# RaphaelHaddad/Real-Time-Brain-Inspired-Video-Memory

Measured on AMD Instinct MI355X. Metric: frame-embeddings/sec (+ kNN queries/sec, see knn), higher is better.
Workload: dtype f16; 1 GPU; BASELINE configs[1]: ViT-B/16-224 encoder fp16, chunks of 16 frames, cosine top-10 over a 100000-row x 768 fp16 memory shard per GPU; chunk_size=16, memory_rows_per_gpu=100000, top_k=10, parallelism=single GPU

## Files before the change

### real-time-brain-inspired-video-memory_amd/csrc/attention.hip

```cpp
#include "vm_internal.h"
#include "vm_kernels.h"

namespace {

typedef short s4v __attribute__((__vector_size__(4 * sizeof(short))));
typedef __attribute__((address_space(3))) s4v *lds_s4v_ptr;
typedef const __attribute__((address_space(3))) char *lds_cptr;

__device__ __forceinline__ bool any_above(const f32x4 a, const f32x4 b, float ref) {
    return (a[0] > ref) | (a[1] > ref) | (a[2] > ref) | (a[3] > ref) | (b[0] > ref) | (b[1] > ref) | (b[2] > ref) |
           (b[3] > ref);
}

template <class E>
__device__ __forceinline__ uint16_t ctx_value(float o, float inv) {
    float prod = o * inv;
    asm("" : "+v"(prod));
    return E::from_float(prod);
}

template <int DT, int NT, bool EXACT, bool CAUSAL = false>
__device__ __forceinline__ void attend_tile(const char *kl, const char *vl, typename vm_elem<DT>::vec8 qa,
                                            typename vm_elem<DT>::vec8 qb, int T, int lane, bool qvalid,
                                            uint16_t *dst_row, int ctx_nt = 0, int qrow = 0) {
    using E = vm_elem<DT>;
    using vec8 = typename E::vec8;
    constexpr int NS = (NT + 1) / 2;
    const int r16 = lane & 15, h = lane >> 4;
    const float scale_log2e = 0.125f * 1.44269504088896340736f;
    const int tq = r16 >> 2, tp = r16 & 3;
    f32x4 s[NT];
    float mx = -INFINITY;
#pragma unroll
    for (int kt = 0; kt < NT; ++kt) {
        const int key = kt * 16 + r16;
        const vec8 k0 = *reinterpret_cast<const vec8 *>(kl + key * 128 + ((h ^ (key & 7)) << 4));
        const vec8 k1 = *reinterpret_cast<const vec8 *>(kl + key * 128 + (((h + 4) ^ (key & 7)) << 4));
        f32x4 a = f32x4{0.f, 0.f, 0.f, 0.f};
        a = E::mfma16(k0, qa, a);
        a = E::mfma16(k1, qb, a);
        if (CAUSAL) {
#pragma unroll
            for (int j = 0; j < 4; ++j) {
                const int key = kt * 16 + 4 * h + j;
                a[j] = (key < T && key <= qrow) ? a[j] : -INFINITY;
            }
        } else if (EXACT ? (kt == NT - 1) : (kt * 16 + 16 > T)) {
#pragma unroll
            for (int j = 0; j < 4; ++j) a[j] = (kt * 16 + 4 * h + j < T) ? a[j] : -INFINITY;
        }
        mx = fmaxf(fmaxf(mx, fmaxf(a[0], a[1])), fmaxf(a[2], a[3]));
        s[kt] = a;
    }
    mx = fmaxf(mx, __shfl_xor(mx, 16, 64));
    mx = fmaxf(mx, __shfl_xor(mx, 32, 64));
    const float neg_mxc = -mx * scale_log2e;
    typedef float f32x2 __attribute__((ext_vector_type(2)));
    const f32x2 c2 = {scale_log2e, scale_log2e}, n2 = {neg_mxc, neg_mxc};
    f32x2 sum2 = {0.f, 0.f};
#pragma unroll
    for (int kt = 0; kt < NT; ++kt) {
        f32x2 a01 = __builtin_elementwise_fma(f32x2{s[kt][0], s[kt][1]}, c2, n2);
        f32x2 a23 = __builtin_elementwise_fma(f32x2{s[kt][2], s[kt][3]}, c2, n2);
        a01 = f32x2{__builtin_amdgcn_exp2f(a01.x), __builtin_amdgcn_exp2f(a01.y)};
        a23 = f32x2{__builtin_amdgcn_exp2f(a23.x), __builtin_amdgcn_exp2f(a23.y)};
        sum2 += a01;
        sum2 += a23;
        s[kt] = f32x4{a01.x, a01.y, a23.x, a23.y};
    }
    float sum = sum2.x + sum2.y;
    sum += __shfl_xor(sum, 16, 64);
    sum += __shfl_xor(sum, 32, 64);
    const float inv = 1.0f / sum;

    f32x4 o[4];
#pragma unroll
    for (int dt = 0; dt < 4; ++dt) o[dt] = f32x4{0.f, 0.f, 0.f, 0.f};
#pragma unroll
    for (int ks = 0; ks < NS; ++ks) {
        uint16_t pe[8];
#pragma unroll
        for (int j = 0; j < 4; ++j) {
            pe[j] = E::from_float(s[2 * ks][j]);
            pe[4 + j] = (2 * ks + 1 < NT) ? E::from_float(s[2 * ks + 1][j]) : (uint16_t)0;
        }
        vec8 pf;
        __builtin_memcpy(&pf, pe, 16);
        const int key_lo = ks * 32 + 4 * h + tq, key_hi = key_lo + 16;
        const char *row_lo = vl + key_lo * 128 + (tp & 1) * 8;
        const int sw = key_lo & 7;
#pragma unroll
        for (int dt = 0; dt < 4; ++dt) {
            const int coff = ((2 * dt + (tp >> 1)) ^ sw) << 4;
            const s4v lo = __builtin_amdgcn_ds_read_tr16_b64_v4i16((lds_s4v_ptr)(row_lo + coff));
            const s4v hi = __builtin_amdgcn_ds_read_tr16_b64_v4i16(
                (lds_s4v_ptr)(row_lo + (2 * ks + 1 < NT ? 16 * 128 : 0) + coff));
            typedef short s8v __attribute__((__vector_size__(8 * sizeof(short))));
            const s8v av = __builtin_shufflevector(lo, hi, 0, 1, 2, 3, 4, 5, 6, 7);
            o[dt] = E::mfma16(__builtin_bit_cast(vec8, av), pf, o[dt]);
        }
        (void)key_hi;
    }
    if (qvalid) {
        uint16_t *dst = dst_row + 4 * h;
#pragma unroll
        for (int dt = 0; dt < 4; ++dt) {
            uint16_t oe[4];
#pragma unroll
            for (int j = 0; j < 4; ++j) oe[j] = ctx_value<E>(o[dt][j], inv);
            uint2 pk;
            __builtin_memcpy(&pk, oe, 8);
            typedef unsigned ctx_u32x2 __attribute__((ext_vector_type(2)));
            if (ctx_nt) __builtin_nontemporal_store(ctx_u32x2{pk.x, pk.y}, reinterpret_cast<ctx_u32x2 *>(dst + dt * 16));
            else *reinterpret_cast<uint2 *>(dst + dt * 16) = pk;
        }
    }
}

template <int DT, int NT, bool EXACT>
__device__ __forceinline__ float attend_rowmax(const char *kl, typename vm_elem<DT>::vec8 qa,
                                               typename vm_elem<DT>::vec8 qb, int T, int lane) {
    using E = vm_elem<DT>;
    using vec8 = typename E::vec8;
    const int r16 = lane & 15, h = lane >> 4;
    const char *p0 = kl + r16 * 128 + ((h ^ (r16 & 7)) << 4);
    const char *p1 = kl + r16 * 128 + (((h + 4) ^ (r16 & 7)) << 4);
    auto tile = [&](int kt, bool masked) {
        const vec8 k0 = *reinterpret_cast<const vec8 *>(p0 + kt * 2048);
        const vec8 k1 = *reinterpret_cast<const vec8 *>(p1 + kt * 2048);
        f32x4 a = f32x4{0.f, 0.f, 0.f, 0.f};
        a = E::mfma16(k0, qa, a);
        a = E::mfma16(k1, qb, a);
        if (masked) {
#pragma unroll
            for (int j = 0; j < 4; ++j) a[j] = (kt * 16 + 4 * h + j < T) ? a[j] : -INFINITY;
        }
        return fmaxf(fmaxf(a[0], a[1]), fmaxf(a[2], a[3]));
    };
    float mx0 = -INFINITY, mx1 = -INFINITY;
    constexpr int FULL = EXACT ? NT - 1 : 0;
    int kt = 0;
#pragma unroll 1
    for (; kt + 1 < FULL; kt += 2) {
        mx0 = fmaxf(mx0, tile(kt, false));
        mx1 = fmaxf(mx1, tile(kt + 1, false));
    }
#pragma unroll 1
    for (; kt < NT; ++kt) mx0 = fmaxf(mx0, tile(kt, kt >= FULL));
    float mx = fmaxf(mx0, mx1);
    mx = fmaxf(mx, __shfl_xor(mx, 16, 64));
    mx = fmaxf(mx, __shfl_xor(mx, 32, 64));
    return mx;
}

template <int DT, int NT, bool EXACT, bool ONLINE = false>
__device__ __forceinline__ void attend_tile_pass2(const char *kl, const char *vl, typename vm_elem<DT>::vec8 qa,
                                                  typename vm_elem<DT>::vec8 qb, float mx, int T, int lane,
                                                  bool qvalid, uint16_t *dst_row) {
    using E = vm_elem<DT>;
    using vec8 = typename E::vec8;
    typedef float f32x2 __attribute__((ext_vector_type(2)));
    typedef short s8v __attribute__((__vector_size__(8 * sizeof(short))));
    constexpr int NS = (NT + 1) / 2;
    const int r16 = lane & 15, h = lane >> 4;
    const int tq = r16 >> 2, tp = r16 & 3;
    const float scale_log2e = 0.125f * 1.44269504088896340736f;
    constexpr float ONLINE_SLACK = 6.0f;
    float run_m = ONLINE ? -1e30f : mx;
    float run_hi = -1e30f;
    float neg_mxc = -run_m * scale_log2e;
    const f32x2 c2 = {scale_log2e, scale_log2e};
    f32x2 n2 = {neg_mxc, neg_mxc};
    const char *p0 = kl + r16 * 128 + ((h ^ (r16 & 7)) << 4);
    const char *p1 = kl + r16 * 128 + (((h + 4) ^ (r16 & 7)) << 4);
    const int vsw = (4 * h + tq) & 7;
    const char *vrow = vl + (4 * h + tq) * 128 + (tp & 1) * 8;
    int voff[4];
#pragma unroll
    for (int dt = 0; dt < 4; ++dt) voff[dt] = ((2 * dt + (tp >> 1)) ^ vsw) << 4;
    f32x2 sum2 = {0.f, 0.f};
    f32x4 o[4];
#pragma unroll
    for (int dt = 0; dt < 4; ++dt) o[dt] = f32x4{0.f, 0.f, 0.f, 0.f};

    lds_cptr kp0 = (lds_cptr)p0, kp1 = (lds_cptr)p1;
    lds_cptr vp[4];
#pragma unroll
    for (int dt = 0; dt < 4; ++dt) vp[dt] = (lds_cptr)(vrow + voff[dt]);
    auto step = [&](int ks, bool masked0, bool has1, bool masked1) {
        const int hi_off = has1 ? 16 * 128 : 0;
        typedef const __attribute__((address_space(3))) vec8 *lds_vec8_ptr;
        const vec8 ka0 = *(lds_vec8_ptr)(kp0);
        const vec8 ka1 = *(lds_vec8_ptr)(kp1);
        const vec8 kb0 = *(lds_vec8_ptr)(kp0 + (has1 ? 2048 : 0));
        const vec8 kb1 = *(lds_vec8_ptr)(kp1 + (has1 ? 2048 : 0));
        s4v vlo[4], vhi[4];
#pragma unroll
        for (int dt = 0; dt < 4; ++dt) {
            vlo[dt] = __builtin_amdgcn_ds_read_tr16_b64_v4i16((lds_s4v_ptr)(vp[dt]));
            vhi[dt] = __builtin_amdgcn_ds_read_tr16_b64_v4i16((lds_s4v_ptr)(vp[dt] + hi_off));
        }
        kp0 += 4096;
        kp1 += 4096;
#pragma unroll
        for (int dt = 0; dt < 4; ++dt) vp[dt] += 4096;
        asm volatile("" : "+v"(kp0), "+v"(kp1), "+v"(vp[0]), "+v"(vp[1]), "+v"(vp[2]), "+v"(vp[3]));
        f32x4 a[2];
        a[0] = E::mfma16(ka0, qa, f32x4{0.f, 0.f, 0.f, 0.f});
        a[0] = E::mfma16(ka1, qb, a[0]);
        a[1] = E::mfma16(kb0, qa, f32x4{0.f, 0.f, 0.f, 0.f});
        a[1] = E::mfma16(kb1, qb, a[1]);
        if (masked0) {
#pragma unroll
            for (int j = 0; j < 4; ++j) a[0][j] = ((2 * ks) * 16 + 4 * h + j < T) ? a[0][j] : -INFINITY;
        }
        if (!has1) {
            a[1] = f32x4{-INFINITY, -INFINITY, -INFINITY, -INFINITY};
        } else if (masked1) {
#pragma unroll
            for (int j = 0; j < 4; ++j) a[1][j] = ((2 * ks + 1) * 16 + 4 * h + j < T) ? a[1][j] : -INFINITY;
        }
        if (ONLINE) {
            if (__ballot(any_above(a[0], a[1], run_hi)) != 0ull) {
                const float lm_own = fmaxf(fmaxf(fmaxf(a[0][0], a[0][1]), fmaxf(a[0][2], a[0][3])),
                                           fmaxf(fmaxf(a[1][0], a[1][1]), fmaxf(a[1][2], a[1][3])));
                float lm = fmaxf(lm_own, __shfl_xor(lm_own, 16, 64));
                lm = fmaxf(lm, __shfl_xor(lm, 32, 64));
                const float m_new = fmaxf(run_m, lm);
                const float f = __builtin_amdgcn_exp2f((run_m - m_new) * scale_log2e);
                sum2 *= f32x2{f, f};
#pragma unroll
                for (int dt = 0; dt < 4; ++dt) o[dt] *= f32x4{f, f, f, f};
                run_m = m_new;
                run_hi = run_m + ONLINE_SLACK / scale_log2e;
                neg_mxc = -run_m * scale_log2e;
                n2 = f32x2{neg_mxc, neg_mxc};
            }
        }
        uint16_t pe[8];
#pragma unroll
        for (int u = 0; u < 2; ++u) {
            f32x2 p01 = __builtin_elementwise_fma(f32x2{a[u][0], a[u][1]}, c2, n2);
            f32x2 p23 = __builtin_elementwise_fma(f32x2{a[u][2], a[u][3]}, c2, n2);
            p01 = f32x2{__builtin_amdgcn_exp2f(p01.x), __builtin_amdgcn_exp2f(p01.y)};
            p23 = f32x2{__builtin_amdgcn_exp2f(p23.x), __builtin_amdgcn_exp2f(p23.y)};
            sum2 += p01 + p23;
            pe[4 * u + 0] = E::from_float(p01.x);
            pe[4 * u + 1] = E::from_float(p01.y);
            pe[4 * u + 2] = E::from_float(p23.x);
            pe[4 * u + 3] = E::from_float(p23.y);
        }
        vec8 pf;
        __builtin_memcpy(&pf, pe, 16);
#pragma unroll
        for (int dt = 0; dt < 4; ++dt) {
            const s8v av = __builtin_shufflevector(vlo[dt], vhi[dt], 0, 1, 2, 3, 4, 5, 6, 7);
            o[dt] = E::mfma16(__builtin_bit_cast(vec8, av), pf, o[dt]);
        }
    };
    constexpr int FULL_STEPS = EXACT ? (NT - 1) / 2 : 0;
    int ks = 0;
#pragma unroll 1
    for (; ks < FULL_STEPS; ++ks) step(ks, false, true, false);
#pragma unroll 1
    for (; ks < NS; ++ks) step(ks, true, 2 * ks + 1 < NT, true);

    float sum = sum2.x + sum2.y;
    sum += __shfl_xor(sum, 16, 64);
    sum += __shfl_xor(sum, 32, 64);
    const float inv = 1.0f / sum;
    if (qvalid) {
        uint16_t *dst = dst_row + 4 * h;
#pragma unroll
        for (int dt = 0; dt < 4; ++dt) {
            uint16_t oe[4];
#pragma unroll
            for (int j = 0; j < 4; ++j) oe[j] = ctx_value<E>(o[dt][j], inv);
            uint2 pk;
            __builtin_memcpy(&pk, oe, 8);
            *reinterpret_cast<uint2 *>(dst + dt * 16) = pk;
        }
    }
}

__device__ __forceinline__ void wait_vmcnt_dyn(int n) {
#define VM_W(N) case N: asm volatile("s_waitcnt vmcnt(" #N ")" ::: "memory"); break;
    switch (n) {
        VM_W(1) VM_W(2) VM_W(3) VM_W(4) VM_W(5) VM_W(6) VM_W(7) VM_W(8) VM_W(9) VM_W(10) VM_W(11) VM_W(12) VM_W(13)
        VM_W(14) VM_W(15) VM_W(16) VM_W(17) VM_W(18) VM_W(19) VM_W(20) VM_W(21) VM_W(22) VM_W(23) VM_W(24) VM_W(25)
        VM_W(26) VM_W(27) VM_W(28) VM_W(29) VM_W(30) VM_W(31) VM_W(32) VM_W(33) VM_W(34) VM_W(35) VM_W(36) VM_W(37)
        VM_W(38) VM_W(39) VM_W(40) VM_W(41) VM_W(42) VM_W(43) VM_W(44) VM_W(45) VM_W(46) VM_W(47) VM_W(48)
        default: asm volatile("s_waitcnt vmcnt(0)" ::: "memory"); break;
    }
#undef VM_W
}

template <int DT, int NT, bool EXACT, int ABL = 0>
__device__ __forceinline__ void attend_pair_online(const char *kl, const char *vl,
                                                   const typename vm_elem<DT>::vec8 (&qa)[2],
                                                   const typename vm_elem<DT>::vec8 (&qb)[2], int T, int lane,
                                                   const bool (&qvalid)[2], uint16_t *const (&dst_row)[2]) {
    using E = vm_elem<DT>;
    using vec8 = typename E::vec8;
    typedef float f32x2 __attribute__((ext_vector_type(2)));
    constexpr int NS = (NT + 1) / 2;
    constexpr float ONLINE_SLACK = 6.0f;
    const int r16 = lane & 15, h = lane >> 4;
    const int tq = r16 >> 2, tp = r16 & 3;
    const float scale_log2e = 0.125f * 1.44269504088896340736f;
    const f32x2 c2 = {scale_log2e, scale_log2e};
    const char *p0 = kl + r16 * 128 + ((h ^ (r16 & 7)) << 4);
    const char *p1 = kl + r16 * 128 + (((h + 4) ^ (r16 & 7)) << 4);
    const int vsw = (4 * h + tq) & 7;
    const char *vrow = vl + (4 * h + tq) * 128 + (tp & 1) * 8;
    int voff[4];
#pragma unroll
    for (int dt = 0; dt < 4; ++dt) voff[dt] = ((2 * dt + (tp >> 1)) ^ vsw) << 4;
    float run_m[2] = {-1e30f, -1e30f}, run_hi[2] = {-1e30f, -1e30f};
    f32x2 n2[2] = {{1e30f * scale_log2e, 1e30f * scale_log2e}, {1e30f * scale_log2e, 1e30f * scale_log2e}};
    f32x2 sum2[2] = {{0.f, 0.f}, {0.f, 0.f}};
    f32x4 o[2][4];
#pragma unroll
    for (int t = 0; t < 2; ++t)
#pragma unroll
        for (int dt = 0; dt < 4; ++dt) o[t][dt] = f32x4{0.f, 0.f, 0.f, 0.f};

    lds_cptr kp0 = (lds_cptr)p0, kp1 = (lds_cptr)p1;
    lds_cptr vp[4];
#pragma unroll
    for (int dt = 0; dt < 4; ++dt) vp[dt] = (lds_cptr)(vrow + voff[dt]);
    auto step = [&](int ks, bool masked0, bool has1, bool masked1) {
        const int hi_off = has1 ? 16 * 128 : 0;
        typedef const __attribute__((address_space(3))) vec8 *lds_vec8_ptr;
        vec8 ka0, ka1, kb0, kb1;
        if (ABL & 32) {
            ka0 = ka1 = qa[0];
            kb0 = kb1 = qb[0];
        } else {
            ka0 = *(lds_vec8_ptr)(kp0);
            ka1 = *(lds_vec8_ptr)(kp1);
            kb0 = *(lds_vec8_ptr)(kp0 + (has1 ? 2048 : 0));
            kb1 = *(lds_vec8_ptr)(kp1 + (has1 ? 2048 : 0));
        }
        s4v vlo[4], vhi[4];
#pragma unroll
        for (int dt = 0; dt < 4; ++dt) {
            if (ABL & 16) {
                vlo[dt] = vhi[dt] = __builtin_bit_cast(s4v, (unsigned long long)(0x3c003c003c003c00ull + dt));
            } else {
                vlo[dt] = __builtin_amdgcn_ds_read_tr16_b64_v4i16((lds_s4v_ptr)(vp[dt]));
                vhi[dt] = __builtin_amdgcn_ds_read_tr16_b64_v4i16((lds_s4v_ptr)(vp[dt] + hi_off));
            }
        }
        kp0 += 4096;
        kp1 += 4096;
#pragma unroll
        for (int dt = 0; dt < 4; ++dt) vp[dt] += 4096;
        asm volatile("" : "+v"(kp0), "+v"(kp1), "+v"(vp[0]), "+v"(vp[1]), "+v"(vp[2]), "+v"(vp[3]));
        f32x4 a[2][2];
        bool out_of_slack = false;
#pragma unroll
        for (int t = 0; t < 2; ++t) {
            if (ABL & 8) {
                const f32x4 ua = __builtin_bit_cast(f32x4, ka0), ub = __builtin_bit_cast(f32x4, kb0);
                a[t][0] = f32x4{1.f, 2.f, 3.f, 4.f} + f32x4{ua[0] * 0.f, 0.f, 0.f, 0.f};
                a[t][1] = f32x4{4.f, 3.f, 2.f, 1.f} + f32x4{ub[0] * 0.f, 0.f, 0.f, 0.f};
                asm volatile("" : "+v"(a[t][0]), "+v"(a[t][1]) : "v"(ka1), "v"(kb1));
            } else {
                a[t][0] = E::mfma16(ka0, qa[t], f32x4{0.f, 0.f, 0.f, 0.f});
                a[t][0] = E::mfma16(ka1, qb[t], a[t][0]);
                a[t][1] = E::mfma16(kb0, qa[t], f32x4{0.f, 0.f, 0.f, 0.f});
                a[t][1] = E::mfma16(kb1, qb[t], a[t][1]);
            }
        }
#pragma unroll
        for (int t = 0; t < 2; ++t) {
            if (masked0) {
#pragma unroll
                for (int j = 0; j < 4; ++j) a[t][0][j] = ((2 * ks) * 16 + 4 * h + j < T) ? a[t][0][j] : -INFINITY;
            }
            if (!has1) {
                a[t][1] = f32x4{-INFINITY, -INFINITY, -INFINITY, -INFINITY};
            } else if (masked1) {
#pragma unroll
                for (int j = 0; j < 4; ++j) a[t][1][j] = ((2 * ks + 1) * 16 + 4 * h + j < T) ? a[t][1][j] : -INFINITY;
            }
            out_of_slack |= any_above(a[t][0], a[t][1], run_hi[t]);
        }
        if (__ballot(out_of_slack) != 0ull) {
#pragma unroll
            for (int t = 0; t < 2; ++t) {
                const float lm_own = fmaxf(fmaxf(fmaxf(a[t][0][0], a[t][0][1]), fmaxf(a[t][0][2], a[t][0][3])),
                                           fmaxf(fmaxf(a[t][1][0], a[t][1][1]), fmaxf(a[t][1][2], a[t][1][3])));
                float lm = fmaxf(lm_own, __shfl_xor(lm_own, 16, 64));
                lm = fmaxf(lm, __shfl_xor(lm, 32, 64));
                const float m_new = lm > run_hi[t] ? lm : run_m[t];
                const float f = __builtin_amdgcn_exp2f((run_m[t] - m_new) * scale_log2e);
                sum2[t] *= f32x2{f, f};
#pragma unroll
                for (int dt = 0; dt < 4; ++dt) o[t][dt] *= f32x4{f, f, f, f};
                run_m[t] = m_new;
                run_hi[t] = m_new + ONLINE_SLACK / scale_log2e;
                const float neg = -m_new * scale_log2e;
                n2[t] = f32x2{neg, neg};
            }
        }
        auto softmax_pack = [&](int t) -> vec8 {
            uint16_t pe[8];
#pragma unroll
            for (int u = 0; u < 2; ++u) {
                f32x2 p01 = __builtin_elementwise_fma(f32x2{a[t][u][0], a[t][u][1]}, c2, n2[t]);
                f32x2 p23 = __builtin_elementwise_fma(f32x2{a[t][u][2], a[t][u][3]}, c2, n2[t]);
                if (!(ABL & 1)) {
                    p01 = f32x2{__builtin_amdgcn_exp2f(p01.x), __builtin_amdgcn_exp2f(p01.y)};
                    p23 = f32x2{__builtin_amdgcn_exp2f(p23.x), __builtin_amdgcn_exp2f(p23.y)};
                }
                sum2[t] += p01 + p23;
                pe[4 * u + 0] = E::from_float(p01.x);
                pe[4 * u + 1] = E::from_float(p01.y);
                pe[4 * u + 2] = E::from_float(p23.x);
                pe[4 * u + 3] = E::from_float(p23.y);
            }
            vec8 pf;
            __builtin_memcpy(&pf, pe, 16);
            return pf;
        };
        vec8 av[4];
#pragma unroll
        for (int dt = 0; dt < 4; ++dt)
            av[dt] = __builtin_bit_cast(vec8, __builtin_shufflevector(vlo[dt], vhi[dt], 0, 1, 2, 3, 4, 5, 6, 7));
        const vec8 pf0 = softmax_pack(0);
        if (ABL & 2) {
            asm volatile("" ::"v"(pf0), "v"(av[0]), "v"(av[1]), "v"(av[2]), "v"(av[3]));
        } else {
#pragma unroll
            for (int dt = 0; dt < 4; ++dt) o[0][dt] = E::mfma16(av[dt], pf0, o[0][dt]);
        }
        const vec8 pf1 = softmax_pack(1);
        if (ABL & 2) {
            asm volatile("" ::"v"(pf1));
        } else {
#pragma unroll
            for (int dt = 0; dt < 4; ++dt) o[1][dt] = E::mfma16(av[dt], pf1, o[1][dt]);
        }
#pragma unroll
        for (int k = 0; k < 4; ++k) {
            __builtin_amdgcn_sched_group_barrier(0x008, 1, 0);
            __builtin_amdgcn_sched_group_barrier(0x400, 2, 0);
        }
    };
    constexpr int FULL_STEPS = EXACT ? (NT - 1) / 2 : 0;
    int ks = 0;
#pragma unroll 1
    for (; ks < FULL_STEPS; ++ks) step(ks, false, true, false);
#pragma unroll 1
    for (; ks < NS; ++ks) step(ks, true, 2 * ks + 1 < NT, true);

#pragma unroll
    for (int t = 0; t < 2; ++t) {
        float sum = sum2[t].x + sum2[t].y;
        sum += __shfl_xor(sum, 16, 64);
        sum += __shfl_xor(sum, 32, 64);
        const float inv = 1.0f / sum;
        if (qvalid[t]) {
            uint16_t *dst = dst_row[t] + 4 * h;
#pragma unroll
            for (int dt = 0; dt < 4; ++dt) {
                uint16_t oe[4];
#pragma unroll
                for (int j = 0; j < 4; ++j) oe[j] = ctx_value<E>(o[t][dt][j], inv);
                uint2 pk;
                __builtin_memcpy(&pk, oe, 8);
                *reinterpret_cast<uint2 *>(dst + dt * 16) = pk;
            }
        }
    }
}

template <int DT, int NT, bool EXACT, int NW, int ABL = 0>
__global__ void __launch_bounds__(NW * 64, 1)
    attention_pair_kernel(const uint16_t *__restrict__ qkv, uint16_t *__restrict__ ctx_out, int T, int heads,
                          int qt_lim) {
    using E = vm_elem<DT>;
    using vec8 = typename E::vec8;
    constexpr int ROWS = NT * 16;
    extern __shared__ __attribute__((aligned(16))) char smem[];
    char *kl = smem, *vl = smem + (size_t)ROWS * 128;
    const int tid = threadIdx.x, lane = tid & 63, wave = tid >> 6;
    const int r16 = lane & 15, h = lane >> 4;
    const int b = blockIdx.x / heads, head = blockIdx.x - b * heads;
    const int H = heads * 64;
    const size_t M = (size_t)(gridDim.x / heads) * T;
    auto block = [&](int part) { return qkv + ((size_t)(part * heads + head) * M + (size_t)b * T) * 64; };
    auto load_q = [&](int qt, vec8 &q0, vec8 &q1) {
        int qtok = qt * 16 + r16;
        if (qtok > T - 1) qtok = T - 1;
        const uint16_t *qp = block(0) + (size_t)qtok * 64;
        q0 = __builtin_bit_cast(vec8, *reinterpret_cast<const uint4 *>(qp + 8 * h));
        q1 = __builtin_bit_cast(vec8, *reinterpret_cast<const uint4 *>(qp + 32 + 8 * h));
    };
    const int srow = lane >> 3, scp = lane & 7;
    auto stage = [&](int part, char *dst) {
        const char *src = reinterpret_cast<const char *>(block(part));
#pragma unroll 4
        for (int grp = wave; grp < ROWS / 8; grp += NW) {
            int key = grp * 8 + srow;
            key = key > T - 1 ? T - 1 : key;
            __builtin_amdgcn_global_load_lds((gbl_ptr_t)(src + (size_t)key * 128 + ((scp ^ srow) << 4)),
                                             (lds_ptr_t)(dst + grp * 1024), 16, 0, 2);
        }
    };
    const int npairs = (qt_lim + 1) / 2;
    vec8 qa[2], qb[2];
    if (wave < npairs) {
        load_q(2 * wave, qa[0], qb[0]);
        load_q(2 * wave + 1, qa[1], qb[1]);
    }
    if (!(ABL & 4)) {
        stage(1, kl);
        stage(2, vl);
    }
    asm volatile("s_waitcnt vmcnt(0)" ::: "memory");
    __syncthreads();
    for (int pr = wave; pr < npairs; pr += NW) {
        bool qvalid[2];
        uint16_t *dst[2];
#pragma unroll
        for (int t = 0; t < 2; ++t) {
            const int qt = 2 * pr + t;
            const int qtok = qt * 16 + r16;
            qvalid[t] = qt < qt_lim && qtok < T;
            dst[t] = ctx_out + ((size_t)b * T + (qvalid[t] ? qtok : 0)) * H + head * 64;
        }
        const vec8 ca[2] = {qa[0], qa[1]}, cb[2] = {qb[0], qb[1]};
        if (pr + NW < npairs) {
            load_q(2 * (pr + NW), qa[0], qb[0]);
            load_q(2 * (pr + NW) + 1, qa[1], qb[1]);
        }
        attend_pair_online<DT, NT, EXACT, ABL>(kl, vl, ca, cb, T, lane, qvalid, dst);
    }
}

template <int DT, int NT, bool EXACT, int NW, int PF_MAX>
__global__ void __launch_bounds__(NW * 64, 1)
    attention_pair_persist_kernel(const uint16_t *__restrict__ qkv, uint16_t *__restrict__ ctx_out, int T, int heads,
                                  int qt_lim, int items) {
    using E = vm_elem<DT>;
    using vec8 = typename E::vec8;
    constexpr int ROWS = NT * 16;
    constexpr int CHUNKS = 2 * ROWS * 8;
    extern __shared__ __attribute__((aligned(16))) char smem[];
    char *kl = smem, *vl = smem + (size_t)ROWS * 128;
    const int tid = threadIdx.x, lane = tid & 63;
    const int wave = __builtin_amdgcn_readfirstlane(tid >> 6);
    const int r16 = lane & 15, h = lane >> 4;
    const int H = heads * 64;
    const size_t M = (size_t)(items / heads) * T;
    if ((int)blockIdx.x >= items) return;
    auto block = [&](int item, int part) {
        const int b = item / heads, head = item - b * heads;
        return qkv + ((size_t)(part * heads + head) * M + (size_t)b * T) * 64;
    };
    auto load_q = [&](int item, int qt, vec8 &q0, vec8 &q1) {
        int qtok = qt * 16 + r16;
        if (qtok > T - 1) qtok = T - 1;
        const uint16_t *qp = block(item, 0) + (size_t)qtok * 64;
        q0 = __builtin_bit_cast(vec8, *reinterpret_cast<const uint4 *>(qp + 8 * h));
        q1 = __builtin_bit_cast(vec8, *reinterpret_cast<const uint4 *>(qp + 32 + 8 * h));
    };
    const int npairs = (qt_lim + 1) / 2;
    const int maxc = (npairs + NW - 1) / NW;
    int w0 = npairs - (maxc - 1) * NW;
    if (w0 >= NW) w0 = 0;
    const int P = NW - w0, pw = wave - w0;

    int item = blockIdx.x;
    vec8 qa[2], qb[2];
    if (wave < npairs) {
        load_q(item, 2 * wave, qa[0], qb[0]);
        load_q(item, 2 * wave + 1, qa[1], qb[1]);
    }
    {
        const int srow = lane >> 3, scp = lane & 7;
#pragma unroll
        for (int part = 1; part <= 2; ++part) {
            const char *src = reinterpret_cast<const char *>(block(item, part));
            char *dst = part == 1 ? kl : vl;
#pragma unroll 4
            for (int grp = wave; grp < ROWS / 8; grp += NW) {
                int key = grp * 8 + srow;
                key = key > T - 1 ? T - 1 : key;
                __builtin_amdgcn_global_load_lds((gbl_ptr_t)(src + (size_t)key * 128 + ((scp ^ srow) << 4)),
                                                 (lds_ptr_t)(dst + grp * 1024), 16, 0, 2);
            }
        }
        asm volatile("s_waitcnt vmcnt(0)" ::: "memory");
        __syncthreads();
    }
    while (true) {
        const int next = item + (int)gridDim.x;
        const bool has_next = next < items;
        const int b = item / heads, head = item - b * heads;
        for (int pr = wave; pr < npairs; pr += NW) {
            bool qvalid[2];
            uint16_t *dst[2];
#pragma unroll
            for (int t = 0; t < 2; ++t) {
                const int qt = 2 * pr + t;
                const int qtok = qt * 16 + r16;
                qvalid[t] = qt < qt_lim && qtok < T;
                dst[t] = ctx_out + ((size_t)b * T + (qvalid[t] ? qtok : 0)) * H + head * 64;
            }
            const vec8 ca[2] = {qa[0], qa[1]}, cb[2] = {qb[0], qb[1]};
            if (pr + NW < npairs) {
                load_q(item, 2 * (pr + NW), qa[0], qb[0]);
                load_q(item, 2 * (pr + NW) + 1, qa[1], qb[1]);
            } else if (has_next && pw < 0) {
                load_q(next, 2 * wave, qa[0], qb[0]);
                load_q(next, 2 * wave + 1, qa[1], qb[1]);
            }
            attend_pair_online<DT, NT, EXACT, 0>(kl, vl, ca, cb, T, lane, qvalid, dst);
        }
        if (!has_next) break;
        if (pw >= 0) {
            typedef unsigned pf_u32x4 __attribute__((ext_vector_type(4)));
            pf_u32x4 buf[PF_MAX];
            const char *kbase = reinterpret_cast<const char *>(block(next, 1));
            const char *vbase = reinterpret_cast<const char *>(block(next, 2));
            int lrow = lane >> 3;
            asm volatile("" : "+v"(lrow));
            const unsigned lane_term = (unsigned)(((lane & 7) ^ lrow) << 4);
#pragma unroll
            for (int j = 0; j < PF_MAX; ++j) {
                int g = __builtin_amdgcn_readfirstlane(j * P + pw);
                g = g < CHUNKS / 64 ? g : CHUNKS / 64 - 1;
                const bool is_v = g >= ROWS / 8;
                int key = (is_v ? g - ROWS / 8 : g) * 8 + lrow;
                key = key > T - 1 ? T - 1 : key;
                const char *src = (is_v ? vbase : kbase) + ((unsigned)key * 128u + lane_term);
                buf[j] = __builtin_nontemporal_load(reinterpret_cast<const pf_u32x4 *>(src));
            }
            asm volatile("s_waitcnt lgkmcnt(0)\n\ts_barrier" ::: "memory");
#pragma unroll
            for (int j = 0; j < PF_MAX; ++j) {
                int g = __builtin_amdgcn_readfirstlane(j * P + pw);
                g = g < CHUNKS / 64 ? g : CHUNKS / 64 - 1;
                *reinterpret_cast<pf_u32x4 *>(smem + (size_t)g * 1024 + lane * 16) = buf[j];
            }
            if (wave < npairs) {
                load_q(next, 2 * wave, qa[0], qb[0]);
                load_q(next, 2 * wave + 1, qa[1], qb[1]);
            }
            asm volatile("s_waitcnt lgkmcnt(0)\n\ts_barrier" ::: "memory");
        } else {
            asm volatile("s_waitcnt lgkmcnt(0)\n\ts_barrier" ::: "memory");
            asm volatile("s_waitcnt lgkmcnt(0)\n\ts_barrier" ::: "memory");
        }
        item = next;
    }
}

template <int DT, int NT, bool EXACT, int NW, bool ONLINE>
__global__ void __launch_bounds__(NW * 64, 1)
    attention_long_kernel(const uint16_t *__restrict__ qkv, uint16_t *__restrict__ ctx_out, int T, int heads,
                          int qt_lim) {
    using E = vm_elem<DT>;
    using vec8 = typename E::vec8;
    constexpr int ROWS = NT * 16;
    extern __shared__ __attribute__((aligned(16))) char smem[];
    char *kl = smem, *vl = smem + (size_t)ROWS * 128;

    const int tid = threadIdx.x, lane = tid & 63, wave = tid >> 6;
    const int r16 = lane & 15, h = lane >> 4;
    const int b = blockIdx.x / heads, head = blockIdx.x - b * heads;
    const int H = heads * 64;
    const size_t M = (size_t)(gridDim.x / heads) * T;
    auto block = [&](int part) { return qkv + ((size_t)(part * heads + head) * M + (size_t)b * T) * 64; };
    auto load_q = [&](int qt, vec8 &q0, vec8 &q1) {
        int qtok = qt * 16 + r16;
        if (qtok > T - 1) qtok = T - 1;
        const uint16_t *qp = block(0) + (size_t)qtok * 64;
        q0 = __builtin_bit_cast(vec8, *reinterpret_cast<const uint4 *>(qp + 8 * h));
        q1 = __builtin_bit_cast(vec8, *reinterpret_cast<const uint4 *>(qp + 32 + 8 * h));
    };
    const int srow = lane >> 3, scp = lane & 7;
    auto stage = [&](int part, char *dst) {
        const char *src = reinterpret_cast<const char *>(block(part));
#pragma unroll 4
        for (int grp = wave; grp < ROWS / 8; grp += NW) {
            int key = grp * 8 + srow;
            key = key > T - 1 ? T - 1 : key;
            __builtin_amdgcn_global_load_lds((gbl_ptr_t)(src + (size_t)key * 128 + ((scp ^ srow) << 4)),
                                             (lds_ptr_t)(dst + grp * 1024), 16, 0, 2);
        }
    };
    vec8 q0, q1;
    load_q(wave, q0, q1);
    stage(1, kl);
    asm volatile("s_waitcnt vmcnt(0)" ::: "memory");
    __syncthreads();
    stage(2, vl);
    float mx = 0.f;
    if (!ONLINE && wave < qt_lim) mx = attend_rowmax<DT, NT, EXACT>(kl, q0, q1, T, lane);
    asm volatile("s_waitcnt vmcnt(0)" ::: "memory");
    __syncthreads();
    for (int qt = wave; qt < qt_lim; qt += NW) {
        const int qtok = qt * 16 + r16;
        const bool qvalid = qtok < T;
        const vec8 qa = q0, qb = q1;
        if (qt + NW < qt_lim) load_q(qt + NW, q0, q1);
        if (!ONLINE && qt != wave) mx = attend_rowmax<DT, NT, EXACT>(kl, qa, qb, T, lane);
        attend_tile_pass2<DT, NT, EXACT, ONLINE>(kl, vl, qa, qb, mx, T, lane, qvalid,
                                         ctx_out + ((size_t)b * T + (qvalid ? qtok : 0)) * H + head * 64);
    }
}

template <int DT, int NT, bool EXACT>
int launch_long(vm_ctx *ctx, const uint16_t *qkv, uint16_t *out, int B, int T, int heads, hipStream_t st, int qt_lim) {
    const size_t lds = (size_t)NT * 16 * 128 * 2;
    static const int online_env = (int)VM_DEV_ENV("ATTN_ONLINE", 1);
    static const int pair_env = (int)VM_DEV_ENV("ATTN_PAIR", 12);
    vm_prof_scope prof(ctx, VM_PROF_ATTENTION, st);
    if (online_env && pair_env > 0) {
        const int ql = qt_lim < NT ? qt_lim : NT;
#define VM_PAIR_GO(NWV)                                                                                              \
    {                                                                                                                \
        auto kern = attention_pair_kernel<DT, NT, EXACT, NWV>;                                                       \
        static unsigned long long attr_set = 0;                                               \
        if (!((attr_set >> (ctx->device & 63)) & 1ull)) {                                                                                             \
            VM_HIP(ctx, hipFuncSetAttribute((const void *)kern, hipFuncAttributeMaxDynamicSharedMemorySize, (int)lds)); \
            attr_set |= 1ull << (ctx->device & 63);                                                                                         \
        }                                                                                                            \
        kern<<<B * heads, NWV * 64, lds, st>>>(qkv, out, T, heads, ql);                                              \
    }
#ifdef VM_DEV_SWITCHES
        static const int abl_env = (int)VM_DEV_ENV("ATTN_ABL", 0);
#define VM_PAIR_ABL(A)                                                                                               \
    if (abl_env == (A)) {                                                                                            \
        auto kern = attention_pair_kernel<DT, NT, EXACT, 12, (A)>;                                                   \
        (void)hipFuncSetAttribute((const void *)kern, hipFuncAttributeMaxDynamicSharedMemorySize, (int)lds);        \
        kern<<<B * heads, 12 * 64, lds, st>>>(qkv, out, T, heads, ql);                                               \
        VM_LAUNCH_CHECK(ctx);                                                                                        \
        return VM_OK;                                                                                                \
    }
        if constexpr (NT == 37 && DT == VM_BF16) {
            VM_PAIR_ABL(1) VM_PAIR_ABL(2) VM_PAIR_ABL(4) VM_PAIR_ABL(8) VM_PAIR_ABL(16) VM_PAIR_ABL(32) VM_PAIR_ABL(3)
            VM_PAIR_ABL(10) VM_PAIR_ABL(48) VM_PAIR_ABL(63)
        }
#undef VM_PAIR_ABL
#endif
        static const int persist_env = (int)VM_DEV_ENV("ATTN_PERSIST", 1);
        const int npairs = (ql + 1) / 2, maxc = (npairs + 11) / 12;
        int w0 = npairs - (maxc - 1) * 12;
        if (w0 >= 12) w0 = 0;
        constexpr int GROUPS = 2 * NT * 16 / 8;
        constexpr int PF_FEW = (GROUPS + 4) / 5;
        constexpr int PF_MANY = (GROUPS + 10) / 11;
        const int pf = (GROUPS + (12 - w0) - 1) / (12 - w0);
        const int items = B * heads;
#define VM_PERSIST_GO(PF)                                                                                            \
    {                                                                                                                \
        auto kern = attention_pair_persist_kernel<DT, NT, EXACT, 12, PF>;                                            \
        static unsigned long long attr_set = 0;                                               \
        if (!((attr_set >> (ctx->device & 63)) & 1ull)) {                                                            \
            VM_HIP(ctx, hipFuncSetAttribute((const void *)kern, hipFuncAttributeMaxDynamicSharedMemorySize, (int)lds)); \
            attr_set |= 1ull << (ctx->device & 63);                                                                  \
        }                                                                                                            \
        kern<<<items < ctx->num_cus ? items : ctx->num_cus, 12 * 64, lds, st>>>(qkv, out, T, heads, ql, items);      \
    }
        if (persist_env && pair_env == 12 && pf <= PF_MANY) VM_PERSIST_GO(PF_MANY)
        else if (persist_env && pair_env == 12 && pf <= PF_FEW) VM_PERSIST_GO(PF_FEW)
#undef VM_PERSIST_GO
        else if (pair_env == 8) VM_PAIR_GO(8)
        else if (pair_env == 10) VM_PAIR_GO(10)
        else VM_PAIR_GO(12)
#undef VM_PAIR_GO
    } else if (online_env) {
        auto kern = attention_long_kernel<DT, NT, EXACT, 16, true>;
        static unsigned long long attr_set = 0;
        if (!((attr_set >> (ctx->device & 63)) & 1ull)) {
            VM_HIP(ctx, hipFuncSetAttribute((const void *)kern, hipFuncAttributeMaxDynamicSharedMemorySize, (int)lds));
            attr_set |= 1ull << (ctx->device & 63);
        }
        kern<<<B * heads, 1024, lds, st>>>(qkv, out, T, heads, qt_lim < NT ? qt_lim : NT);
    } else {
        auto kern = attention_long_kernel<DT, NT, EXACT, 16, false>;
        static unsigned long long attr_set = 0;
        if (!((attr_set >> (ctx->device & 63)) & 1ull)) {
            VM_HIP(ctx, hipFuncSetAttribute((const void *)kern, hipFuncAttributeMaxDynamicSharedMemorySize, (int)lds));
            attr_set |= 1ull << (ctx->device & 63);
        }
        kern<<<B * heads, 1024, lds, st>>>(qkv, out, T, heads, qt_lim < NT ? qt_lim : NT);
    }
    VM_LAUNCH_CHECK(ctx);
    return VM_OK;
}

template <int DT, int NT, bool EXACT, int OCC, bool CAUSAL = false>
__global__ void __launch_bounds__(256, OCC)
    attention_kernel(const uint16_t *__restrict__ qkv, uint16_t *__restrict__ ctx_out, int T, int heads, int qt_lim) {
    using E = vm_elem<DT>;
    using vec8 = typename E::vec8;
    constexpr int KROWS = NT * 16;
    constexpr int VROWS = KROWS;
    extern __shared__ __attribute__((aligned(16))) char smem[];
    char *kl = smem;
    char *vl = smem + (size_t)KROWS * 128;

    const int tid = threadIdx.x, lane = tid & 63, wave = tid >> 6;
    const int r16 = lane & 15, h = lane >> 4;
    const int b = blockIdx.x / heads, head = blockIdx.x - b * heads;
    const int H = heads * 64;
    const size_t M = (size_t)(gridDim.x / heads) * T;
    auto block = [&](int part) { return qkv + ((size_t)(part * heads + head) * M + (size_t)b * T) * 64; };

    auto load_q = [&](int qt, vec8 &q0, vec8 &q1) {
        int qtok = qt * 16 + r16;
        if (qtok > T - 1) qtok = T - 1;
        const uint16_t *qp = block(0) + (size_t)qtok * 64;
        q0 = __builtin_bit_cast(vec8, *reinterpret_cast<const uint4 *>(qp + 8 * h));
        q1 = __builtin_bit_cast(vec8, *reinterpret_cast<const uint4 *>(qp + 32 + 8 * h));
    };
    vec8 q0, q1;
    load_q(wave, q0, q1);
    {
        constexpr int GROUPS = (KROWS + VROWS) / 8;
        const int srow = lane >> 3, scp = lane & 7;
#pragma unroll
        for (int gi = 0; gi < (GROUPS + 3) / 4; ++gi) {
            const int grp = gi * 4 + wave;
            if (grp < GROUPS) {
                const int r = grp * 8 + srow;
                const bool is_v = r >= KROWS;
                int key = is_v ? r - KROWS : r;
                if (key > T - 1) key = T - 1;
                const uint16_t *src = block(is_v ? 2 : 1) + (size_t)key * 64 + ((scp ^ (r & 7)) << 3);
                __builtin_amdgcn_global_load_lds((gbl_ptr_t)src, (lds_ptr_t)(smem + grp * 1024), 16, 0, 0);
            }
        }
        asm volatile("s_waitcnt vmcnt(0)" ::: "memory");
    }
    __syncthreads();

    for (int qt = wave; qt < qt_lim; qt += 4) {
        const int qtok = qt * 16 + r16;
        const bool qvalid = qtok < T;
        const vec8 qa = q0, qb = q1;
        if (qt + 4 < qt_lim) load_q(qt + 4, q0, q1);

        attend_tile<DT, NT, EXACT, CAUSAL>(kl, vl, qa, qb, T, lane, qvalid,
                                           ctx_out + ((size_t)b * T + (qvalid ? qtok : 0)) * H + head * 64, 0, qtok);
    }
}

template <int DT, int NT, bool EXACT, int CW>
__global__ void __launch_bounds__((CW + 1) * 64, 1)
    attention_stream_kernel(const uint16_t *__restrict__ qkv, uint16_t *__restrict__ ctx_out, int T, int heads,
                            int items, int qt_lim, int ctx_nt) {
    using E = vm_elem<DT>;
    using vec8 = typename E::vec8;
    constexpr int ROWS = NT * 16;
    constexpr int IMG = 3 * ROWS * 128;
    constexpr int QT = (NT + CW - 1) / CW;
    extern __shared__ __attribute__((aligned(16))) char smem[];

    const int tid = threadIdx.x, lane = tid & 63, wave = tid >> 6;
    const int H = heads * 64;
    if (blockIdx.x >= items) return;

    if (wave == CW) {
        const int srow = lane >> 3, scp = lane & 7;
        const unsigned lane_off = (unsigned)((scp ^ srow) << 4);
        const size_t M = (size_t)(items / heads) * T;
        const int tmax = T - 1;
        int buf = 0;
        for (int item = blockIdx.x; item < items; item += gridDim.x, buf ^= 1) {
            const int b = item / heads, head = item - b * heads;
#pragma unroll
            for (int part = 0; part < 3; ++part) {
                const char *pbase = reinterpret_cast<const char *>(
                    qkv + ((size_t)((part == 2 ? 0 : part + 1) * heads + head) * M + (size_t)b * T) * 64);
#pragma unroll
                for (int g = 0; g < ROWS / 8; ++g) {
                    if (part == 2 && g >= 2 * qt_lim) break;
                    int key = g * 8 + srow;
                    if (!EXACT || g * 8 + 7 >= 16 * (NT - 1)) key = key > tmax ? tmax : key;
                    const unsigned off = (unsigned)key * 128 + lane_off;
                    __builtin_amdgcn_global_load_lds((gbl_ptr_t)(pbase + off),
                                                     (lds_ptr_t)(smem + buf * IMG + (part * (ROWS / 8) + g) * 1024), 16,
                                                     0, 2);
                    if ((g & 3) == 3) asm volatile("s_waitcnt vmcnt(24)" ::: "memory");
                }
            }
            asm volatile("s_waitcnt vmcnt(0)" ::: "memory");
            asm volatile("s_barrier" ::: "memory");
        }
        return;
    }

    const int r16 = lane & 15, h = lane >> 4;
    int buf = 0;
    for (int item = blockIdx.x; item < items; item += gridDim.x, buf ^= 1) {
        asm volatile("s_barrier" ::: "memory");
        const char *kl = smem + buf * IMG, *vl = kl + ROWS * 128, *ql = vl + ROWS * 128;
        const int b = item / heads, head = item - b * heads;
#pragma unroll
        for (int u = 0; u < QT; ++u) {
            const int qt = wave + CW * u;
            if (qt < qt_lim) {
                const int qtok = qt * 16 + r16;
                const bool qvalid = qtok < T;
                const vec8 qa = *reinterpret_cast<const vec8 *>(ql + qtok * 128 + ((h ^ (qtok & 7)) << 4));
                const vec8 qb = *reinterpret_cast<const vec8 *>(ql + qtok * 128 + (((h + 4) ^ (qtok & 7)) << 4));
                attend_tile<DT, NT, EXACT>(kl, vl, qa, qb, T, lane, qvalid,
                                           ctx_out + ((size_t)b * T + (qvalid ? qtok : 0)) * H + head * 64, ctx_nt);
            }
        }
    }
}

template <int DT, int NT, bool EXACT, int CW>
int launch_stream_cw(vm_ctx *ctx, const uint16_t *qkv, uint16_t *out, int B, int T, int heads, hipStream_t st, int qt_lim) {
    const size_t lds = (size_t)NT * 16 * 128 * 6;
    auto kern = attention_stream_kernel<DT, NT, EXACT, CW>;
    static unsigned long long attr_set = 0;
    if (!((attr_set >> (ctx->device & 63)) & 1ull)) {
        VM_HIP(ctx, hipFuncSetAttribute((const void *)kern, hipFuncAttributeMaxDynamicSharedMemorySize, (int)lds));
        attr_set |= 1ull << (ctx->device & 63);
    }
    const int items = B * heads;
    const int grid = items < ctx->num_cus ? items : ctx->num_cus;
    vm_prof_scope prof(ctx, VM_PROF_ATTENTION, st);
    static const int ctx_nt_env = (int)VM_DEV_ENV("ATTN_CTX_NT", 1);
    kern<<<grid, (CW + 1) * 64, lds, st>>>(qkv, out, T, heads, items, qt_lim < NT ? qt_lim : NT, ctx_nt_env);
    VM_LAUNCH_CHECK(ctx);
    return VM_OK;
}

template <int DT, int NT, bool EXACT>
int launch_stream(vm_ctx *ctx, const uint16_t *qkv, uint16_t *out, int B, int T, int heads, hipStream_t st, int qt_lim) {
    static const int cw_env = (int)VM_DEV_ENV("ATTN_CW", 13);
    if (cw_env == 8) return launch_stream_cw<DT, NT, EXACT, 8>(ctx, qkv, out, B, T, heads, st, qt_lim);
    return launch_stream_cw<DT, NT, EXACT, 13>(ctx, qkv, out, B, T, heads, st, qt_lim);
}


template <int DT, int NT, bool EXACT, int OCC = (NT <= 13 ? 2 : 1), bool CAUSAL = false>
int launch(vm_ctx *ctx, const uint16_t *qkv, uint16_t *out, int B, int T, int heads, hipStream_t st, int qt_lim) {
    const size_t lds = (size_t)NT * 16 * 128 * 2;
    auto kern = attention_kernel<DT, NT, EXACT, OCC, CAUSAL>;
    static unsigned long long attr_set = 0;
    if (!((attr_set >> (ctx->device & 63)) & 1ull)) {
        VM_HIP(ctx, hipFuncSetAttribute((const void *)kern, hipFuncAttributeMaxDynamicSharedMemorySize, (int)lds));
        attr_set |= 1ull << (ctx->device & 63);
    }
    vm_prof_scope prof(ctx, VM_PROF_ATTENTION, st);
    kern<<<B * heads, 256, lds, st>>>(qkv, out, T, heads, qt_lim < NT ? qt_lim : NT);
    VM_LAUNCH_CHECK(ctx);
    return VM_OK;
}

template <int DT>
int dispatch(vm_ctx *ctx, const uint16_t *qkv, uint16_t *out, int B, int T, int heads, hipStream_t st, int q_rows,
             int causal) {
    const int nt = (T + 15) / 16;
    if (causal) {
        if (nt > 5) return vm_fail(ctx, VM_ERR_UNSUPPORTED, "causal attention: %d tokens > 80", T);
        return launch<DT, 5, false, 2, true>(ctx, qkv, out, B, T, heads, st, 5);
    }
    const int ql = q_rows > 0 ? (q_rows + 15) / 16 : nt;
    if (nt == 13) {
        return launch_stream<DT, 13, true>(ctx, qkv, out, B, T, heads, st, ql);
    }
    if (nt == 37) return launch_long<DT, 37, true>(ctx, qkv, out, B, T, heads, st, ql);
    if (nt <= 2) return launch<DT, 2, false>(ctx, qkv, out, B, T, heads, st, ql);
    if (nt <= 5) return launch<DT, 5, false>(ctx, qkv, out, B, T, heads, st, ql);
    if (nt <= 13) return launch<DT, 13, false>(ctx, qkv, out, B, T, heads, st, ql);
    if (nt <= 37) return launch_long<DT, 37, false>(ctx, qkv, out, B, T, heads, st, ql);
    return vm_fail(ctx, VM_ERR_UNSUPPORTED, "attention: %d tokens > 592", T);
}

}

int vm_attention(vm_ctx *ctx, int dtype, const uint16_t *qkv, uint16_t *ctx_out, int B, int T, int heads,
                 hipStream_t st, int q_rows, int causal) {
    return dtype == VM_F16 ? dispatch<VM_F16>(ctx, qkv, ctx_out, B, T, heads, st, q_rows, causal)
                           : dispatch<VM_BF16>(ctx, qkv, ctx_out, B, T, heads, st, q_rows, causal);
}
```

Measured before the change: 26600 frame-embeddings/s.

## Stage attention context in LDS and drain it from the producer wave

The streaming attention kernel's producer wave now fills only K and V into LDS. Each compute wave loads its own Q tile straight from global memory, prefetching the next item's Q. Compute waves write their context output into a swizzled LDS staging buffer instead of global memory. The producer wave then drains that buffer to global with coalesced 16-byte stores while it fills the next item, and the vmcnt throttling window during fill becomes a template parameter that defaults to off. The aim is to cut scattered 8-byte global stores from the compute waves and overlap output writeback with the next load, at the cost of one wave doing both load and store work plus extra barriers.

```diff
diff --git a/real-time-brain-inspired-video-memory_amd/csrc/attention.hip b/real-time-brain-inspired-video-memory_amd/csrc/attention.hip
--- a/real-time-brain-inspired-video-memory_amd/csrc/attention.hip
+++ b/real-time-brain-inspired-video-memory_amd/csrc/attention.hip
@@ -19,7 +19,7 @@
     return E::from_float(prod);
 }
 
-template <int DT, int NT, bool EXACT, bool CAUSAL = false>
+template <int DT, int NT, bool EXACT, bool CAUSAL = false, bool LDS_CTX = false>
 __device__ __forceinline__ void attend_tile(const char *kl, const char *vl, typename vm_elem<DT>::vec8 qa,
                                             typename vm_elem<DT>::vec8 qb, int T, int lane, bool qvalid,
                                             uint16_t *dst_row, int ctx_nt = 0, int qrow = 0) {
@@ -111,6 +111,12 @@
             uint2 pk;
             __builtin_memcpy(&pk, oe, 8);
             typedef unsigned ctx_u32x2 __attribute__((ext_vector_type(2)));
+            if constexpr (LDS_CTX) {
+                typedef __attribute__((address_space(3))) ctx_u32x2 *lds_ctx_ptr;
+                char *row = reinterpret_cast<char *>(dst_row);
+                *(lds_ctx_ptr)(row + (((2 * dt + (h >> 1)) ^ (qrow & 7)) << 4) + (h & 1) * 8) = ctx_u32x2{pk.x, pk.y};
+                continue;
+            }
             if (ctx_nt) __builtin_nontemporal_store(ctx_u32x2{pk.x, pk.y}, reinterpret_cast<ctx_u32x2 *>(dst + dt * 16));
             else *reinterpret_cast<uint2 *>(dst + dt * 16) = pk;
         }
@@ -853,76 +859,121 @@
     }
 }
 
-template <int DT, int NT, bool EXACT, int CW>
+template <int DT, int NT, bool EXACT, int CW, int WIN>
 __global__ void __launch_bounds__((CW + 1) * 64, 1)
     attention_stream_kernel(const uint16_t *__restrict__ qkv, uint16_t *__restrict__ ctx_out, int T, int heads,
                             int items, int qt_lim, int ctx_nt) {
     using E = vm_elem<DT>;
     using vec8 = typename E::vec8;
     constexpr int ROWS = NT * 16;
-    constexpr int IMG = 3 * ROWS * 128;
-    constexpr int QT = (NT + CW - 1) / CW;
+    constexpr int IMG = 2 * ROWS * 128;
+    constexpr int CIMG = ROWS * 128;
+    static_assert(NT <= CW, "one query tile per compute wave");
+    static_assert(WIN >= 0 && WIN < 64, "the window must fit the vmcnt field");
     extern __shared__ __attribute__((aligned(16))) char smem[];
+    typedef unsigned st_u32x4 __attribute__((ext_vector_type(4)));
 
     const int tid = threadIdx.x, lane = tid & 63, wave = tid >> 6;
     const int H = heads * 64;
     if (blockIdx.x >= items) return;
+    const size_t M = (size_t)(items / heads) * T;
 
     if (wave == CW) {
         const int srow = lane >> 3, scp = lane & 7;
         const unsigned lane_off = (unsigned)((scp ^ srow) << 4);
-        const size_t M = (size_t)(items / heads) * T;
         const int tmax = T - 1;
-        int buf = 0;
-        for (int item = blockIdx.x; item < items; item += gridDim.x, buf ^= 1) {
+        const int row_lim = qt_lim * 16 < T ? qt_lim * 16 : T;
+        auto fill = [&](int item, int buf) {
             const int b = item / heads, head = item - b * heads;
 #pragma unroll
-            for (int part = 0; part < 3; ++part) {
+            for (int part = 0; part < 2; ++part) {
                 const char *pbase = reinterpret_cast<const char *>(
-                    qkv + ((size_t)((part == 2 ? 0 : part + 1) * heads + head) * M + (size_t)b * T) * 64);
+                    qkv + ((size_t)((part + 1) * heads + head) * M + (size_t)b * T) * 64);
 #pragma unroll
                 for (int g = 0; g < ROWS / 8; ++g) {
-                    if (part == 2 && g >= 2 * qt_lim) break;
                     int key = g * 8 + srow;
                     if (!EXACT || g * 8 + 7 >= 16 * (NT - 1)) key = key > tmax ? tmax : key;
                     const unsigned off = (unsigned)key * 128 + lane_off;
                     __builtin_amdgcn_global_load_lds((gbl_ptr_t)(pbase + off),
                                                      (lds_ptr_t)(smem + buf * IMG + (part * (ROWS / 8) + g) * 1024), 16,
                                                      0, 2);
-                    if ((g & 3) == 3) asm volatile("s_waitcnt vmcnt(24)" ::: "memory");
+                    if (WIN > 0 && (g & 3) == 3) asm volatile("s_waitcnt vmcnt(%0)" ::"n"(WIN) : "memory");
                 }
             }
-            asm volatile("s_waitcnt vmcnt(0)" ::: "memory");
-            asm volatile("s_barrier" ::: "memory");
-        }
+        };
+        auto drain = [&](int item, int buf) {
+            const int b = item / heads, head = item - b * heads;
+            int grp_bytes = H * 16;
+            asm volatile("" : "+s"(grp_bytes));
+            char *obase = reinterpret_cast<char *>(ctx_out + ((size_t)b * T * H + (size_t)head * 64));
+            const unsigned lane_dst = (unsigned)srow * ((unsigned)grp_bytes >> 3) + lane_off;
+            const char *img = smem + 2 * IMG + buf * CIMG + lane * 16;
+            constexpr int GB = NT;
+            for (int g0 = 0; g0 < 2 * GB && g0 * 8 < row_lim; g0 += GB) {
+                st_u32x4 v[GB];
+#pragma unroll
+                for (int j = 0; j < GB; ++j)
+                    v[j] = *reinterpret_cast<const __attribute__((address_space(3))) st_u32x4 *>(
+                        (lds_cptr)(img + (g0 + j) * 1024));
+#pragma unroll
+                for (int j = 0; j < GB; ++j) {
+                    if ((g0 + j) * 8 + srow < row_lim) {
+                        st_u32x4 *dst = reinterpret_cast<st_u32x4 *>(obase + (size_t)(g0 + j) * grp_bytes + lane_dst);
+                        if (ctx_nt) __builtin_nontemporal_store(v[j], dst);
+                        else *dst = v[j];
+                    }
+                }
+            }
+        };
+        const int n = (items - (int)blockIdx.x + (int)gridDim.x - 1) / (int)gridDim.x;
+        fill(blockIdx.x, 0);
+        asm volatile("s_waitcnt vmcnt(0)\n\ts_barrier" ::: "memory");
+        for (int k = 0; k < n; ++k) {
+            const int item = blockIdx.x + k * gridDim.x;
+            if (k > 0) drain(item - (int)gridDim.x, (k - 1) & 1);
+            if (k + 1 < n) fill(item + (int)gridDim.x, (k + 1) & 1);
+            asm volatile("s_waitcnt vmcnt(0)\n\ts_barrier" ::: "memory");
+        }
+        drain(blockIdx.x + (n - 1) * gridDim.x, (n - 1) & 1);
         return;
     }
 
     const int r16 = lane & 15, h = lane >> 4;
+    const bool mine = wave < qt_lim;
+    const int qtok = wave * 16 + r16;
+    const bool qvalid = qtok < T;
+    const int qrow = qtok > T - 1 ? T - 1 : qtok;
+    auto load_q = [&](int item, st_u32x4 &q0, st_u32x4 &q1) {
+        const int b = item / heads, head = item - b * heads;
+        const uint16_t *qp = qkv + ((size_t)head * M + (size_t)b * T + qrow) * 64 + 8 * h;
+        q0 = *reinterpret_cast<const st_u32x4 *>(qp);
+        q1 = *reinterpret_cast<const st_u32x4 *>(qp + 32);
+    };
+    st_u32x4 q0 = {}, q1 = {};
+    if (mine) load_q(blockIdx.x, q0, q1);
     int buf = 0;
     for (int item = blockIdx.x; item < items; item += gridDim.x, buf ^= 1) {
-        asm volatile("s_barrier" ::: "memory");
-        const char *kl = smem + buf * IMG, *vl = kl + ROWS * 128, *ql = vl + ROWS * 128;
-        const int b = item / heads, head = item - b * heads;
-#pragma unroll
-        for (int u = 0; u < QT; ++u) {
-            const int qt = wave + CW * u;
-            if (qt < qt_lim) {
-                const int qtok = qt * 16 + r16;
-                const bool qvalid = qtok < T;
-                const vec8 qa = *reinterpret_cast<const vec8 *>(ql + qtok * 128 + ((h ^ (qtok & 7)) << 4));
-                const vec8 qb = *reinterpret_cast<const vec8 *>(ql + qtok * 128 + (((h + 4) ^ (qtok & 7)) << 4));
-                attend_tile<DT, NT, EXACT>(kl, vl, qa, qb, T, lane, qvalid,
-                                           ctx_out + ((size_t)b * T + (qvalid ? qtok : 0)) * H + head * 64, ctx_nt);
-            }
-        }
-    }
-}
-
-template <int DT, int NT, bool EXACT, int CW>
-int launch_stream_cw(vm_ctx *ctx, const uint16_t *qkv, uint16_t *out, int B, int T, int heads, hipStream_t st, int qt_lim) {
+        asm volatile("s_waitcnt lgkmcnt(0)\n\ts_barrier" ::: "memory");
+        if (mine) {
+            const char *kl = smem + buf * IMG, *vl = kl + ROWS * 128;
+            char *crow = smem + 2 * IMG + buf * CIMG + qtok * 128;
+            const vec8 qa = __builtin_bit_cast(vec8, q0), qb = __builtin_bit_cast(vec8, q1);
+            const int next = item + (int)gridDim.x;
+            if (next < items) load_q(next, q0, q1);
+            attend_tile<DT, NT, EXACT, false, true>(kl, vl, qa, qb, T, lane, qvalid,
+                                                    reinterpret_cast<uint16_t *>(crow), 0, qtok);
+        }
+    }
+    asm volatile("s_waitcnt lgkmcnt(0)\n\ts_barrier" ::: "memory");
+}
+
+constexpr int STREAM_WIN = 0;
+
+template <int DT, int NT, bool EXACT, int WIN>
+int launch_stream_win(vm_ctx *ctx, const uint16_t *qkv, uint16_t *out, int B, int T, int heads, hipStream_t st, int qt_lim) {
+    constexpr int CW = 13;
     const size_t lds = (size_t)NT * 16 * 128 * 6;
-    auto kern = attention_stream_kernel<DT, NT, EXACT, CW>;
+    auto kern = attention_stream_kernel<DT, NT, EXACT, CW, WIN>;
     static unsigned long long attr_set = 0;
     if (!((attr_set >> (ctx->device & 63)) & 1ull)) {
         VM_HIP(ctx, hipFuncSetAttribute((const void *)kern, hipFuncAttributeMaxDynamicSharedMemorySize, (int)lds));
@@ -939,9 +990,16 @@
 
 template <int DT, int NT, bool EXACT>
 int launch_stream(vm_ctx *ctx, const uint16_t *qkv, uint16_t *out, int B, int T, int heads, hipStream_t st, int qt_lim) {
-    static const int cw_env = (int)VM_DEV_ENV("ATTN_CW", 13);
-    if (cw_env == 8) return launch_stream_cw<DT, NT, EXACT, 8>(ctx, qkv, out, B, T, heads, st, qt_lim);
-    return launch_stream_cw<DT, NT, EXACT, 13>(ctx, qkv, out, B, T, heads, st, qt_lim);
+#ifdef VM_DEV_SWITCHES
+    const int win_env = (int)VM_DEV_ENV("ATTN_WIN", STREAM_WIN);
+    if (win_env != STREAM_WIN) {
+        if (win_env == 0) return launch_stream_win<DT, NT, EXACT, 0>(ctx, qkv, out, B, T, heads, st, qt_lim);
+        if (win_env == 24) return launch_stream_win<DT, NT, EXACT, 24>(ctx, qkv, out, B, T, heads, st, qt_lim);
+        if (win_env == 40) return launch_stream_win<DT, NT, EXACT, 40>(ctx, qkv, out, B, T, heads, st, qt_lim);
+        if (win_env == 56) return launch_stream_win<DT, NT, EXACT, 56>(ctx, qkv, out, B, T, heads, st, qt_lim);
+    }
+#endif
+    return launch_stream_win<DT, NT, EXACT, STREAM_WIN>(ctx, qkv, out, B, T, heads, st, qt_lim);
 }
 
 
@@ -969,6 +1027,11 @@
         return launch<DT, 5, false, 2, true>(ctx, qkv, out, B, T, heads, st, 5);
     }
     const int ql = q_rows > 0 ? (q_rows + 15) / 16 : nt;
+#ifdef VM_DEV_SWITCHES
+    static const int stream_env = (int)VM_DEV_ENV("ATTN_STREAM", -1);
+    if (stream_env == 0 && nt == 13) return launch<DT, 13, true>(ctx, qkv, out, B, T, heads, st, ql);
+    if (stream_env == 1 && nt < 13) return launch_stream<DT, 13, false>(ctx, qkv, out, B, T, heads, st, ql);
+#endif
     if (nt == 13) {
         return launch_stream<DT, 13, true>(ctx, qkv, out, B, T, heads, st, ql);
     }
```

New measurement: 26670 frame-embeddings/s, median of 6. About the same (+0.2%).
